# vpariza/open-hummingbird-eval

Measured on AMD Instinct MI355X. Metric: query-patches/sec, higher is better.
Workload: dtype f32

## Files before the change

### open-hummingbird-eval_amd/csrc/hbird_knn_f16.hip

```cpp
#include "hbird_knn_dev.h"
#include "hbird_rerank_dev.h"
#include <algorithm>

typedef _Float16 f16x8 __attribute__((ext_vector_type(8)));


__global__ __launch_bounds__(256) void tiles_to_f16_kernel(const float* __restrict__ t32, int g8, _Float16* __restrict__ t16,
                                                           int g16, int64_t n_row_tiles, int64_t rt0, int* __restrict__ overflow) {
    const int64_t gid = (int64_t)blockIdx.x * 256 + threadIdx.x;
    const int64_t total = n_row_tiles * g16 * 64;
    if (gid >= total) return;
    const int i = (int)(gid & 31), h = (int)((gid >> 5) & 1);
    const int64_t blk = gid >> 6;
    const int g = (int)(blk % g16);
    const int64_t rt = rt0 + blk / g16;
    f16x8 out;
#pragma unroll
    for (int j = 0; j < 8; ++j) {
        const int k = 16 * g + 8 * h + j;
        const int gg = k >> 3, kk = k & 7;
        float v = 0.0f;
        if (gg < g8) v = t32[((rt * g8) + gg) * HB_BLK + ((kk & 1) * 32 + i) * 4 + (kk >> 1)];
        out[j] = (_Float16)v;
        if (overflow && fabsf(v) > 65504.0f && fabsf(v) < INFINITY) *overflow = 1;
    }
    reinterpret_cast<f16x8*>(t16)[(rt * g16 + g) * 64 + h * 32 + i] = out;
}

int hb_launch_tiles_to_f16(const float* t32, int g8, _Float16* t16, int g16, int64_t n_row_tiles, int64_t rt0, int* overflow,
                           hipStream_t s) {
    const int64_t total = n_row_tiles * g16 * 64;
    if (total == 0) return 0;
    tiles_to_f16_kernel<<<dim3((unsigned)((total + 255) / 256)), dim3(256), 0, s>>>(t32, g8, t16, g16, n_row_tiles, rt0, overflow);
    HB_HIP(hipGetLastError());
    return 0;
}

#define F2_RING 8
#define F2_SLOT 16384
#define F2_BINIT (F2_RING * F2_SLOT)
#define F2_SCRATCH (F2_BINIT + 2048)
#define F2_PCNT (F2_SCRATCH + 8192)
#define F2_CLWORDS (F2_PCNT + 1024)
#define F2_LDS_TOTAL (F2_CLWORDS + 64)
static_assert(F2_LDS_TOTAL <= 160 * 1024, "LDS budget");

#define F2_DMA(SRC, LDS_ADDR, VOFF)                                                                                          \
    asm volatile("s_mov_b32 m0, %2\n\ts_nop 0\n\tglobal_load_lds_dwordx4 %0, %1" :: "v"(VOFF), "s"(SRC), "s"(LDS_ADDR) : "memory", "m0");
#define F2_BL(REG, SRC, OFF) asm volatile("global_load_dwordx4 %0, %1, %2 offset:" #OFF : "+v"(REG) : "v"(lane_off), "s"(SRC) : "memory");

template <int EMAX>
__global__ __launch_bounds__(HB_THREADS, 2) void knn_f16v2_kernel(knn16_args a) {
    extern __shared__ __attribute__((aligned(16))) char smem[];
    const int tid = threadIdx.x;
    const int lane = tid & 63;
    const int w = __builtin_amdgcn_readfirstlane(tid >> 6);
    const int h = lane >> 5;
    float* sc = reinterpret_cast<float*>(smem + F2_SCRATCH) + w * 256;
    int* pcnt = reinterpret_cast<int*>(smem + F2_PCNT);
    const int g16 = a.g16;
    const int NS = g16 / 2;
    const int myq = w * 32 + (lane & 31);
    const unsigned lane_off = (unsigned)lane * 16u;
    const unsigned lds_0 = (unsigned)(size_t)(__attribute__((address_space(3))) char*)smem;
    const unsigned lds_w = lds_0 + (unsigned)w * 2048u;
    cl_sync cs = cl_init(a.wg_member, a.prog, a.cl, a.lag, blockIdx.x, w == 0, smem + F2_CLWORDS);

    wg_stamp<knn16_args>(0);
    const int seg_begin = a.wg_off[blockIdx.x], seg_end = a.wg_end[blockIdx.x];
    if (w == 0) cl_publish(cs, seg_begin < seg_end ? a.segs[seg_begin].tile0 * NS : 0x7FFFFFFF, lane);
    for (int si = seg_begin; si < seg_end; ++si) {
        const hb_seg seg = HB_KARG(knn16_args, segs)[si];
        const int k = HB_KARG(knn16_args, k), klw = HB_KARG(knn16_args, klw);
        float* wl_s = HB_KARG(knn16_args, state_s) + (size_t)seg.slot * HB_QT * klw;
        unsigned* wl_i = HB_KARG(knn16_args, state_i) + (size_t)seg.slot * HB_QT * klw;
        float thr;
        {
            const knn_args_pool_view pv{HB_KARG(knn16_args, state_cnt), HB_KARG(knn16_args, state_thr)};
            thr = pool_begin(pv, seg.slot, seg.first, pcnt, myq, lane);
            thr = fmaxf(thr, floor_load(HB_KARG(knn16_args, gthr), seg.q_tile * HB_QT + myq));
        }
        const int total = seg.n_tiles * NS, clock0 = seg.tile0 * NS;
        f32x16 acc[8];
        f16x8 fa[8];
        f16x8 bq[4][2];

        const char* const qbase = reinterpret_cast<const char*>(a.q16) + (size_t)(seg.q_tile * 8 + w) * g16 * 1024;
        const char* qf = qbase;
        const char* qf1 = qbase;
        const char* bf = reinterpret_cast<const char*>(a.bank16) + ((size_t)seg.b_tile0 * 8 + w) * g16 * 1024;
        const float* bi = a.binit + (size_t)seg.b_tile0 * HB_BT;
        const long long b_wrap = ((long long)seg.stride * 8 - 1) * g16 * 1024;
        const int bi_step = seg.stride * HB_BT;
        int fks = 0, left = total;
        unsigned slot_f = 0, fpar = 0;
#define F2_REQ_B0(U) F2_BL(bq[U][0], qf, 0)
#define F2_REQ_B1(U) F2_BL(bq[U][1], qf1, 1024)
#define F2_REQ_C(I) F2_DMA(bf, lds_w + slot_f + (I) * 1024u, lane_off + (I) * 1024u)
#define F2_ADVANCE()                                                                                                         \
        {                                                                                                                    \
            if (fks == 0 && w == 0) F2_DMA(bi, lds_0 + F2_BINIT + fpar, lane_off)                                            \
            qf1 = qf;                                                                                                        \
            if (--left > 0) {                                                                                                \
                qf += 2048; bf += 2048;                                                                                      \
                if (++fks == NS) { fks = 0; qf = qbase; bf += b_wrap; bi += bi_step; fpar ^= 1024u; }                        \
            }                                                                                                                \
            slot_f = (slot_f + F2_SLOT) & (F2_RING * F2_SLOT - 1);                                                           \
        }
        F2_REQ_B0(0) F2_REQ_C(0) F2_REQ_C(1) F2_ADVANCE() F2_REQ_B1(0)
        F2_REQ_B0(1) F2_REQ_C(0) F2_REQ_C(1) F2_ADVANCE() F2_REQ_B1(1)
        F2_REQ_B0(2) F2_REQ_C(0) F2_REQ_C(1) F2_ADVANCE() F2_REQ_B1(2)
        F2_REQ_B0(3) F2_REQ_C(0) F2_REQ_C(1) F2_ADVANCE()
        asm volatile("s_waitcnt vmcnt(11)" : "+v"(bq[0][0]), "+v"(bq[0][1]) :: "memory");
        __syncthreads();
        unsigned slot_c = 0;
        int ks = 0, bt = seg.b_tile0, cpar = 0;
        bool bulk = seg.tile0 < 16;
#define F2_INIT_TILE()                                                                                                       \
        {                                                                                                                    \
            const f32x4* bi_ = reinterpret_cast<const f32x4*>(smem + F2_BINIT + cpar * 1024);                                \
            _Pragma("unroll") for (int t = 0; t < 8; ++t)                                                                    \
                _Pragma("unroll") for (int g = 0; g < 4; ++g) {                                                              \
                    const f32x4 v = bi_[8 * t + 2 * g + h];                                                                  \
                    acc[t][4 * g + 0] = v[0]; acc[t][4 * g + 1] = v[1]; acc[t][4 * g + 2] = v[2]; acc[t][4 * g + 3] = v[3]; \
                }                                                                                                            \
        }
        {
            const f16x8* A = reinterpret_cast<const f16x8*>(smem) + lane;
#pragma unroll
            for (int t = 0; t < 8; ++t) fa[t] = A[(t * 2) * 64];
        }
        F2_INIT_TILE()
#define F2_MM(T, B) acc[T] = __builtin_amdgcn_mfma_f32_32x32x16_f16(fa[T], B, acc[T], 0, 0, 0);
#define F2_STAGE(U)                                                                                                          \
        {                                                                                                                    \
            const f16x8* Ac = reinterpret_cast<const f16x8*>(smem + slot_c) + lane;                                          \
            const unsigned slot_n = (slot_c + F2_SLOT) & (F2_RING * F2_SLOT - 1);                                            \
            const f16x8* An = reinterpret_cast<const f16x8*>(smem + slot_n) + lane;                                          \
                                       \
            KN_FENCE F2_MM(0, bq[U][0]) KN_FENCE fa[0] = Ac[(0 * 2 + 1) * 64]; F2_REQ_B1((U + 3) & 3)                           \
            KN_FENCE F2_MM(1, bq[U][0]) KN_FENCE fa[1] = Ac[(1 * 2 + 1) * 64];                                                  \
            KN_FENCE F2_MM(2, bq[U][0]) KN_FENCE fa[2] = Ac[(2 * 2 + 1) * 64];                                                  \
            KN_FENCE F2_MM(3, bq[U][0]) KN_FENCE fa[3] = Ac[(3 * 2 + 1) * 64];                                                  \
            KN_FENCE F2_MM(4, bq[U][0]) KN_FENCE fa[4] = Ac[(4 * 2 + 1) * 64];                                                  \
            KN_FENCE F2_MM(5, bq[U][0]) KN_FENCE fa[5] = Ac[(5 * 2 + 1) * 64];                                                  \
            KN_FENCE F2_MM(6, bq[U][0]) KN_FENCE fa[6] = Ac[(6 * 2 + 1) * 64];                                                  \
            KN_FENCE F2_MM(7, bq[U][0]) KN_FENCE fa[7] = Ac[(7 * 2 + 1) * 64];                                                  \
            KN_FENCE                                                                                                         \
                                \
            asm volatile("s_waitcnt vmcnt(8)" : "+v"(bq[(U + 1) & 3][0]), "+v"(bq[(U + 1) & 3][1]), "+v"(bq[U][1]) :: "memory"); \
            __builtin_amdgcn_s_barrier();      \
                 \
            if ((U) == 0 && w == 0) cl_tick(cs, clock0 + st, lane);    \
            KN_FENCE F2_MM(0, bq[U][1]) KN_FENCE fa[0] = An[(0 * 2) * 64]; F2_REQ_B0(U)                                         \
            KN_FENCE F2_MM(1, bq[U][1]) KN_FENCE fa[1] = An[(1 * 2) * 64];                                                      \
            KN_FENCE F2_MM(2, bq[U][1]) KN_FENCE fa[2] = An[(2 * 2) * 64]; F2_REQ_C(0)                                          \
            KN_FENCE F2_MM(3, bq[U][1]) KN_FENCE fa[3] = An[(3 * 2) * 64];                                                      \
            KN_FENCE F2_MM(4, bq[U][1]) KN_FENCE fa[4] = An[(4 * 2) * 64]; F2_REQ_C(1)                                          \
            KN_FENCE F2_MM(5, bq[U][1]) KN_FENCE fa[5] = An[(5 * 2) * 64];                                                      \
            KN_FENCE F2_MM(6, bq[U][1]) KN_FENCE fa[6] = An[(6 * 2) * 64];                                                      \
            KN_FENCE F2_MM(7, bq[U][1]) KN_FENCE fa[7] = An[(7 * 2) * 64];                                                      \
            KN_FENCE                                                                                                         \
            F2_ADVANCE()                                                                                                     \
            KN_FENCE                                                                                                         \
            slot_c = slot_n;                                                                                                 \
        }
        for (int st = 0; st < total; st += 4) {
            F2_STAGE(0) F2_STAGE(1) F2_STAGE(2) F2_STAGE(3)
            ks += 4;
            if (ks == NS) {
                if (seg.first && bt == seg.b_tile0 && cold_start_needed(thr)) thr = fmaxf(thr, cold_start_threshold(acc, k));
                pool_epilogue_scan<EMAX>(acc, thr, wl_s, wl_i, sc, w * 32, lane, k, (unsigned)bt, klw, pcnt, bulk);
                ks = 0; bt += seg.stride; cpar ^= 1;
                F2_INIT_TILE()
                {
                    const f16x8* A = reinterpret_cast<const f16x8*>(smem + slot_c) + lane;
#pragma unroll
                    for (int t = 0; t < 8; ++t) fa[t] = A[(t * 2) * 64];
                }
            }
        }
        asm volatile("s_waitcnt vmcnt(0)" : "+v"(bq[0][0]), "+v"(bq[0][1]), "+v"(bq[1][0]), "+v"(bq[1][1]), "+v"(bq[2][0]), "+v"(bq[2][1]),
                     "+v"(bq[3][0]), "+v"(bq[3][1]) :: "memory");
#undef F2_STAGE
#undef F2_MM
#undef F2_INIT_TILE
#undef F2_ADVANCE
#undef F2_REQ_B0
#undef F2_REQ_B1
#undef F2_REQ_C
        if (w == 0) cl_publish(cs, seg.next_tile0 == 0x7FFFFFFF ? 0x7FFFFFFF : seg.next_tile0 * NS, lane);
        {
            const knn_args_pool_view pv{HB_KARG(knn16_args, state_cnt), HB_KARG(knn16_args, state_thr)};
            pool_end(pv, seg.slot, pcnt, thr, myq, lane);
        }
        if (lane < 32) floor_publish(HB_KARG(knn16_args, gthr), seg.q_tile * HB_QT + myq, thr);
        asm volatile("s_waitcnt vmcnt(0)" ::: "memory");
        __syncthreads();
    }
    cl_finish(cs, a.cl_stats, w == 0, lane);
    wg_stamp<knn16_args>(1);
}

#define HB_RERANK_PARAMS                                                                                                     \
    const float* __restrict__ binit, int d, const float* __restrict__ q, const float* __restrict__ qn2,                      \
    const int64_t* __restrict__ cand, const float* __restrict__ cand_score, const float* __restrict__ qnorm,                \
    const float* __restrict__ bmax, unsigned char* __restrict__ certified, int kc, int64_t nq, int k, int64_t id_base,      \
    int metric, int out_metric, int64_t ntotal, int64_t* __restrict__ out_idx, float* __restrict__ out_dist,                \
    hb_rerank_seeds sd, hb_centre_view cv

template <bool CENTRED>
__global__ __launch_bounds__(256) void rerank_kernel(const float* __restrict__ tiles, int g8, HB_RERANK_PARAMS) {
    __shared__ float s_sc[4][256];
    __shared__ int64_t s_id[4][256];
    const int lane = threadIdx.x & 63, wv = threadIdx.x >> 6;
    const int64_t qi = (int64_t)blockIdx.x * 4 + wv;
    if (qi >= nq) return;
    const float* qr = q + qi * (int64_t)d;
    const hb_rerank_query qc = hb_rerank_query_of<CENTRED>(qi, qnorm, bmax, d, metric, cv, cand, cand_score, kc, k);
    for (int c = lane; c < kc; c += 64) {
        const int64_t row = cand[qi * (int64_t)kc + c];
        float acc = -INFINITY;
        if (hb_rerank_needs_score(row, c, k, cand_score + qi * (int64_t)kc, qc.cut)) {
            acc = binit[row];
            const float* base = tiles + ((row >> 5) * (int64_t)g8) * HB_BLK + (int)(row & 31) * 4;
            for (int g = 0; g < g8; ++g) {
                const f32x4 e = *reinterpret_cast<const f32x4*>(base + (int64_t)g * HB_BLK);
                const f32x4 o = *reinterpret_cast<const f32x4*>(base + (int64_t)g * HB_BLK + 128);
                const int k0 = 8 * g;
#pragma unroll
                for (int j = 0; j < 4; ++j) {
                    if (k0 + 2 * j < d) acc = fmaf(qr[k0 + 2 * j], e[j], acc);
                    if (k0 + 2 * j + 1 < d) acc = fmaf(qr[k0 + 2 * j + 1], o[j], acc);
                }
            }
        }
        s_sc[wv][c] = acc;
        s_id[wv][c] = row;
    }
    __builtin_amdgcn_s_waitcnt(0xc07f);
    hb_rerank_tail<CENTRED>(s_sc[wv], s_id[wv], lane, qi, qc.E, qc.cq, cand, cand_score, qnorm, qn2, certified, kc, k, id_base, out_metric, ntotal, out_idx, out_dist, sd, cv);
}

__global__ __launch_bounds__(256) void tiles_to_rows_kernel(const float* __restrict__ t32, int g8, float* __restrict__ rows, int rs,
                                                            int64_t rt0) {
    __shared__ float s[4 * HB_BLK];
    const int64_t rt = rt0 + blockIdx.x;
    const int g0 = blockIdx.y * 4, ng = min(4, g8 - g0);
    const int t = threadIdx.x;
    if (t < ng * 64) reinterpret_cast<f32x4*>(s)[t] = reinterpret_cast<const f32x4*>(t32 + (rt * g8 + g0) * HB_BLK)[t];
    __syncthreads();
    const int i = t >> 3, c = t & 7;
    f32x4 out;
#pragma unroll
    for (int j = 0; j < 4; ++j) {
        const int kq = 4 * c + j, gl = kq >> 3, kk = kq & 7;
        out[j] = gl < ng ? s[gl * HB_BLK + ((kk & 1) * 32 + i) * 4 + (kk >> 1)] : 0.0f;
    }
    if (8 * g0 + 4 * c < rs) *reinterpret_cast<f32x4*>(rows + (rt * 32 + i) * (int64_t)rs + 8 * g0 + 4 * c) = out;
}

int hb_launch_tiles_to_row_copy(const float* t32, int g8, float* rows, int rs, int64_t n_row_tiles, int64_t rt0, hipStream_t s) {
    if (n_row_tiles <= 0) return 0;
    tiles_to_rows_kernel<<<dim3((unsigned)n_row_tiles, (unsigned)((rs / 8 + 3) / 4)), dim3(256), 0, s>>>(t32, g8, rows, rs, rt0);
    HB_HIP(hipGetLastError());
    return 0;
}

#define RRW_STRIDE 36
template <bool CENTRED>
__global__ __launch_bounds__(256) void rerank_rows_kernel(const float* __restrict__ rows, int rs, HB_RERANK_PARAMS) {
    __shared__ float s_sc[4][256];
    __shared__ unsigned s_id[4][256];
    __shared__ int s_act[4][256];
    __shared__ __attribute__((aligned(16))) float s_img[4][66 * RRW_STRIDE];
    const int lane = threadIdx.x & 63, wv = threadIdx.x >> 6;
    const int64_t qi = (int64_t)blockIdx.x * 4 + wv;
    if (qi >= nq) return;
    const float* qr = q + qi * (int64_t)d;
    const hb_rerank_query qc = hb_rerank_query_of<CENTRED>(qi, qnorm, bmax, d, metric, cv, cand, cand_score, kc, k);
    int n_act = 0;
    for (int c0 = 0; c0 < kc; c0 += 64) {
        const int c = c0 + lane;
        int64_t row = -1;
        bool act = false;
        if (c < kc) {
            row = cand[qi * (int64_t)kc + c];
            act = hb_rerank_needs_score(row, c, k, cand_score + qi * (int64_t)kc, qc.cut);
            s_sc[wv][c] = -INFINITY;
            s_id[wv][c] = row >= 0 ? (unsigned)row : HB_ID_NONE;
        }
        const unsigned long long m = __ballot(act);
        if (act) s_act[wv][n_act + __popcll(m & ((1ull << lane) - 1ull))] = c;
        n_act += __popcll(m);
    }
    __builtin_amdgcn_s_waitcnt(0xc07f);
    __builtin_amdgcn_wave_barrier();
    float* img = s_img[wv];
    const int rr = lane >> 3, chn = lane & 7;
    const int nch = (d + 31) >> 5;
    for (int b0 = 0; b0 < n_act; b0 += 64) {
        const int nb = min(64, n_act - b0);
        const int nj = (nb + 1 + 7) >> 3;
        const int c = lane < nb ? s_act[wv][b0 + lane] : -1;
        float acc = c >= 0 ? binit[s_id[wv][c]] : 0.0f;
        const float* src[9];
#pragma unroll
        for (int j = 0; j < 9; ++j) {
            const int li = 8 * j + rr;
            src[j] = li < nb ? rows + (int64_t)s_id[wv][s_act[wv][b0 + li]] * rs + 4 * chn : (li == nb ? qr + 4 * chn : nullptr);
        }
        f32x4 R[9];
#define RRW_LOAD(CH)                                                                                                         \
        _Pragma("unroll") for (int j = 0; j < 9; ++j) {                                                                      \
            if (j < nj) {                                                                                                    \
                R[j] = f32x4{0.f, 0.f, 0.f, 0.f};                                                                            \
                if (src[j]) {                                                                                                \
                    const int k0 = 32 * (CH) + 4 * chn;                                                                      \
                    if (8 * j + rr < nb || k0 + 4 <= d) R[j] = *reinterpret_cast<const f32x4*>(src[j] + 32 * (CH));          \
                    else { _Pragma("unroll") for (int e = 0; e < 4; ++e) if (k0 + e < d) R[j][e] = src[j][32 * (CH) + e]; }   \
                }                                                                                                            \
            }                                                                                                                \
        }
        RRW_LOAD(0)
        for (int ch = 0; ch < nch; ++ch) {
#pragma unroll
            for (int j = 0; j < 9; ++j)
                if (j < nj && 8 * j + rr <= nb) *reinterpret_cast<f32x4*>(img + (8 * j + rr) * RRW_STRIDE + 4 * chn) = R[j];
            if (ch + 1 < nch) { RRW_LOAD(ch + 1) }
            __builtin_amdgcn_s_waitcnt(0xc07f);
            __builtin_amdgcn_wave_barrier();
            if (c >= 0) {
                const f32x4* xr = reinterpret_cast<const f32x4*>(img + lane * RRW_STRIDE);
                const f32x4* qv = reinterpret_cast<const f32x4*>(img + nb * RRW_STRIDE);
                if (32 * ch + 32 <= d) {
#pragma unroll
                    for (int i = 0; i < 8; ++i) {
                        const f32x4 x = xr[i], y = qv[i];
                        acc = fmaf(y[0], x[0], acc); acc = fmaf(y[1], x[1], acc); acc = fmaf(y[2], x[2], acc); acc = fmaf(y[3], x[3], acc);
                    }
                } else {
                    for (int i = 0; 32 * ch + i < d; ++i) acc = fmaf(img[nb * RRW_STRIDE + i], img[lane * RRW_STRIDE + i], acc);
                }
            }
            __builtin_amdgcn_wave_barrier();
        }
#undef RRW_LOAD
        if (c >= 0) s_sc[wv][c] = acc;
    }
    __builtin_amdgcn_s_waitcnt(0xc07f);
    __builtin_amdgcn_wave_barrier();
    hb_rerank_tail<CENTRED>(s_sc[wv], s_id[wv], lane, qi, qc.E, qc.cq, cand, cand_score, qnorm, qn2, certified, kc, k, id_base, out_metric, ntotal, out_idx, out_dist, sd, cv);
}
#undef HB_RERANK_PARAMS

int hb_launch_rerank(const hb_rerank_args& a, const float* tiles, int g8, const float* rows, int rs, hipStream_t s) {
    if (a.nq == 0) return 0;
    if (a.kc > 256) return hb_fail("hb_index_search: too many candidates for the re-rank kernel");
    const bool centred = a.cv.cq != nullptr;
    auto fn = rows ? (centred ? rerank_rows_kernel<true> : rerank_rows_kernel<false>) : (centred ? rerank_kernel<true> : rerank_kernel<false>);
    fn<<<dim3((unsigned)((a.nq + 3) / 4)), dim3(256), 0, s>>>(rows ? rows : tiles, rows ? rs : g8, a.binit, a.d, a.q, a.qn2, a.cand, a.cand_score, a.qnorm, a.bmax,
                                                            a.certified, a.kc, a.nq, a.k, a.id_base, a.metric, a.out_metric, a.ntotal, a.out_idx, a.out_dist, a.sd, a.cv);
    HB_HIP(hipGetLastError());
    return 0;
}

int hb_knn_f16_launch(const knn16_args& args, int grid, hipStream_t s) {
    void (*fn)(knn16_args) = args.klw <= 256 ? knn_f16v2_kernel<4> : knn_f16v2_kernel<8>;
    if (args.klw > 512) return hb_fail("hb_index_search: candidate pools beyond 512 entries");
    if (hb_ensure_dyn_lds((const void*)fn, F2_LDS_TOTAL)) return -1;
    fn<<<dim3((unsigned)grid), dim3(HB_THREADS), F2_LDS_TOTAL, s>>>(args);
    HB_HIP(hipGetLastError());
    return 0;
}

__global__ __launch_bounds__(256) void bnorm_max_kernel(const float* __restrict__ bnorm, int64_t n, float* __restrict__ bmax) {
    float m = 0.0f;
    for (int64_t i = (int64_t)blockIdx.x * 256 + threadIdx.x; i < n; i += (int64_t)gridDim.x * 256) m = fmaxf(m, bnorm[i]);
    for (int o = 32; o > 0; o >>= 1) m = fmaxf(m, __shfl_xor(m, o));
    if ((threadIdx.x & 63) == 0) atomicMax(reinterpret_cast<int*>(bmax), __float_as_int(m));
}

int hb_launch_bnorm_max(const float* bnorm, int64_t n, float* bmax, hipStream_t s) {
    if (n == 0) return 0;
    const int64_t blocks = std::min<int64_t>((n + 255) / 256, 1024);
    bnorm_max_kernel<<<dim3((unsigned)blocks), dim3(256), 0, s>>>(bnorm, n, bmax);
    HB_HIP(hipGetLastError());
    return 0;
}

__global__ __launch_bounds__(256) void scatter_rows_kernel(const int64_t* __restrict__ rows, int64_t n, int k,
                                                           const int64_t* __restrict__ src_idx, const float* __restrict__ src_dist,
                                                           int64_t* __restrict__ out_idx, float* __restrict__ out_dist) {
    const int64_t t = (int64_t)blockIdx.x * 256 + threadIdx.x;
    if (t >= n * k) return;
    const int64_t i = t / k;
    const int j = (int)(t % k);
    out_idx[rows[i] * k + j] = src_idx[t];
    out_dist[rows[i] * k + j] = src_dist[t];
}

int hb_launch_scatter_rows(const int64_t* rows, int64_t n, int k, const int64_t* src_idx, const float* src_dist,
                           int64_t* out_idx, float* out_dist, hipStream_t s) {
    if (n == 0) return 0;
    scatter_rows_kernel<<<dim3((unsigned)((n * k + 255) / 256)), dim3(256), 0, s>>>(rows, n, k, src_idx, src_dist, out_idx, out_dist);
    HB_HIP(hipGetLastError());
    return 0;
}
```

Measured before the change: 79270.

## Switch kNN f16 kernel from 32x32x16 to 16x16x32 MFMA with permlane fixup

```diff
diff --git a/open-hummingbird-eval_amd/csrc/hbird_knn_f16.hip b/open-hummingbird-eval_amd/csrc/hbird_knn_f16.hip
--- a/open-hummingbird-eval_amd/csrc/hbird_knn_f16.hip
+++ b/open-hummingbird-eval_amd/csrc/hbird_knn_f16.hip
@@ -47,7 +47,19 @@
 
 #define F2_DMA(SRC, LDS_ADDR, VOFF)                                                                                          \
     asm volatile("s_mov_b32 m0, %2\n\ts_nop 0\n\tglobal_load_lds_dwordx4 %0, %1" :: "v"(VOFF), "s"(SRC), "s"(LDS_ADDR) : "memory", "m0");
-#define F2_BL(REG, SRC, OFF) asm volatile("global_load_dwordx4 %0, %1, %2 offset:" #OFF : "+v"(REG) : "v"(lane_off), "s"(SRC) : "memory");
+#define F2_BL(REG, SRC, OFF) asm volatile("global_load_dwordx4 %0, %1, %2 offset:" #OFF : "+v"(REG) : "v"(q_off), "s"(SRC) : "memory");
+
+template <int Q>
+__device__ __forceinline__ void f2_mm16(f32x16& acc, const f16x8& a, const f16x8& b) {
+    f32x4 c = {acc[4 * Q], acc[4 * Q + 1], acc[4 * Q + 2], acc[4 * Q + 3]};
+    c = __builtin_amdgcn_mfma_f32_16x16x32_f16(a, b, c, 0, 0, 0);
+    acc[4 * Q] = c[0]; acc[4 * Q + 1] = c[1]; acc[4 * Q + 2] = c[2]; acc[4 * Q + 3] = c[3];
+}
+template <int X, int Y>
+__device__ __forceinline__ void f2_swap16(f32x16& acc) {
+    const auto r = __builtin_amdgcn_permlane16_swap(__float_as_uint(acc[X]), __float_as_uint(acc[Y]), false, false);
+    acc[X] = __uint_as_float(r[0]); acc[Y] = __uint_as_float(r[1]);
+}
 
 template <int EMAX>
 __global__ __launch_bounds__(HB_THREADS, 2) void knn_f16v2_kernel(knn16_args a) {
@@ -55,13 +67,16 @@
     const int tid = threadIdx.x;
     const int lane = tid & 63;
     const int w = __builtin_amdgcn_readfirstlane(tid >> 6);
-    const int h = lane >> 5;
+    const int c4 = lane >> 4, m16 = lane & 15;
     float* sc = reinterpret_cast<float*>(smem + F2_SCRATCH) + w * 256;
     int* pcnt = reinterpret_cast<int*>(smem + F2_PCNT);
     const int g16 = a.g16;
     const int NS = g16 / 2;
     const int myq = w * 32 + (lane & 31);
     const unsigned lane_off = (unsigned)lane * 16u;
+    const unsigned q_off = (unsigned)((c4 >> 1) * 1024 + ((c4 & 1) * 32 + m16) * 16);
+    const unsigned a_off = (unsigned)((c4 >> 1) * 1024 + ((c4 & 1) * 32 + 8 * ((m16 >> 2) & 1) + 4 * (m16 >> 3) + (m16 & 3)) * 16);
+    const int ri = 2 * (c4 & 1) + (c4 >> 1);
     const unsigned lds_0 = (unsigned)(size_t)(__attribute__((address_space(3))) char*)smem;
     const unsigned lds_w = lds_0 + (unsigned)w * 2048u;
     cl_sync cs = cl_init(a.wg_member, a.prog, a.cl, a.lag, blockIdx.x, w == 0, smem + F2_CLWORDS);
@@ -87,7 +102,6 @@
 
         const char* const qbase = reinterpret_cast<const char*>(a.q16) + (size_t)(seg.q_tile * 8 + w) * g16 * 1024;
         const char* qf = qbase;
-        const char* qf1 = qbase;
         const char* bf = reinterpret_cast<const char*>(a.bank16) + ((size_t)seg.b_tile0 * 8 + w) * g16 * 1024;
         const float* bi = a.binit + (size_t)seg.b_tile0 * HB_BT;
         const long long b_wrap = ((long long)seg.stride * 8 - 1) * g16 * 1024;
@@ -95,23 +109,22 @@
         int fks = 0, left = total;
         unsigned slot_f = 0, fpar = 0;
 #define F2_REQ_B0(U) F2_BL(bq[U][0], qf, 0)
-#define F2_REQ_B1(U) F2_BL(bq[U][1], qf1, 1024)
+#define F2_REQ_B1(U) F2_BL(bq[U][1], qf, 256)
 #define F2_REQ_C(I) F2_DMA(bf, lds_w + slot_f + (I) * 1024u, lane_off + (I) * 1024u)
 #define F2_ADVANCE()                                                                                                         \
         {                                                                                                                    \
             if (fks == 0 && w == 0) F2_DMA(bi, lds_0 + F2_BINIT + fpar, lane_off)                                            \
-            qf1 = qf;                                                                                                        \
             if (--left > 0) {                                                                                                \
                 qf += 2048; bf += 2048;                                                                                      \
                 if (++fks == NS) { fks = 0; qf = qbase; bf += b_wrap; bi += bi_step; fpar ^= 1024u; }                        \
             }                                                                                                                \
             slot_f = (slot_f + F2_SLOT) & (F2_RING * F2_SLOT - 1);                                                           \
         }
-        F2_REQ_B0(0) F2_REQ_C(0) F2_REQ_C(1) F2_ADVANCE() F2_REQ_B1(0)
-        F2_REQ_B0(1) F2_REQ_C(0) F2_REQ_C(1) F2_ADVANCE() F2_REQ_B1(1)
-        F2_REQ_B0(2) F2_REQ_C(0) F2_REQ_C(1) F2_ADVANCE() F2_REQ_B1(2)
-        F2_REQ_B0(3) F2_REQ_C(0) F2_REQ_C(1) F2_ADVANCE()
-        asm volatile("s_waitcnt vmcnt(11)" : "+v"(bq[0][0]), "+v"(bq[0][1]) :: "memory");
+        F2_REQ_C(0) F2_REQ_C(1) F2_REQ_B0(0) F2_REQ_B1(0) F2_ADVANCE()
+        F2_REQ_C(0) F2_REQ_C(1) F2_REQ_B0(1) F2_REQ_B1(1) F2_ADVANCE()
+        F2_REQ_C(0) F2_REQ_C(1) F2_REQ_B0(2) F2_REQ_B1(2) F2_ADVANCE()
+        F2_REQ_C(0) F2_REQ_C(1) F2_REQ_B0(3) F2_REQ_B1(3) F2_ADVANCE()
+        asm volatile("s_waitcnt vmcnt(12)" : "+v"(bq[0][0]), "+v"(bq[0][1]) :: "memory");
         __syncthreads();
         unsigned slot_c = 0;
         int ks = 0, bt = seg.b_tile0, cpar = 0;
@@ -120,46 +133,53 @@
         {                                                                                                                    \
             const f32x4* bi_ = reinterpret_cast<const f32x4*>(smem + F2_BINIT + cpar * 1024);                                \
             _Pragma("unroll") for (int t = 0; t < 8; ++t)                                                                    \
-                _Pragma("unroll") for (int g = 0; g < 4; ++g) {                                                              \
-                    const f32x4 v = bi_[8 * t + 2 * g + h];                                                                  \
-                    acc[t][4 * g + 0] = v[0]; acc[t][4 * g + 1] = v[1]; acc[t][4 * g + 2] = v[2]; acc[t][4 * g + 3] = v[3]; \
+                _Pragma("unroll") for (int f = 0; f < 2; ++f) {                                                              \
+                    const f32x4 v = bi_[8 * t + 4 * f + ri];                                                                 \
+                    _Pragma("unroll") for (int j = 0; j < 4; ++j) { acc[t][8 * f + j] = v[j]; acc[t][8 * f + 4 + j] = v[j]; } \
                 }                                                                                                            \
         }
+#define F2_SWAP_TILE()                                                                                                       \
+        _Pragma("unroll") for (int t = 0; t < 8; ++t) {                                                                      \
+            f2_swap16<0, 4>(acc[t]); f2_swap16<1, 5>(acc[t]); f2_swap16<2, 6>(acc[t]); f2_swap16<3, 7>(acc[t]);              \
+            f2_swap16<8, 12>(acc[t]); f2_swap16<9, 13>(acc[t]); f2_swap16<10, 14>(acc[t]); f2_swap16<11, 15>(acc[t]);        \
+        }
+#define F2_FRAG(BASE, F) (*reinterpret_cast<const f16x8*>((BASE) + ((F) >> 1) * 2048 + ((F) & 1) * 256))
         {
-            const f16x8* A = reinterpret_cast<const f16x8*>(smem) + lane;
-#pragma unroll
-            for (int t = 0; t < 8; ++t) fa[t] = A[(t * 2) * 64];
+            const char* A = smem + a_off;
+#pragma unroll
+            for (int i = 0; i < 8; ++i) fa[i] = F2_FRAG(A, i);
         }
         F2_INIT_TILE()
-#define F2_MM(T, B) acc[T] = __builtin_amdgcn_mfma_f32_32x32x16_f16(fa[T], B, acc[T], 0, 0, 0);
+#define F2_MM(F, U) f2_mm16<2 * ((F) & 1)>(acc[(F) >> 1], fa[(F) & 7], bq[U][0]); f2_mm16<2 * ((F) & 1) + 1>(acc[(F) >> 1], fa[(F) & 7], bq[U][1]);
 #define F2_STAGE(U)                                                                                                          \
         {                                                                                                                    \
-            const f16x8* Ac = reinterpret_cast<const f16x8*>(smem + slot_c) + lane;                                          \
+            const char* Ac = smem + slot_c + a_off;                                                                          \
             const unsigned slot_n = (slot_c + F2_SLOT) & (F2_RING * F2_SLOT - 1);                                            \
-            const f16x8* An = reinterpret_cast<const f16x8*>(smem + slot_n) + lane;                                          \
-                                       \
-            KN_FENCE F2_MM(0, bq[U][0]) KN_FENCE fa[0] = Ac[(0 * 2 + 1) * 64]; F2_REQ_B1((U + 3) & 3)                           \
-            KN_FENCE F2_MM(1, bq[U][0]) KN_FENCE fa[1] = Ac[(1 * 2 + 1) * 64];                                                  \
-            KN_FENCE F2_MM(2, bq[U][0]) KN_FENCE fa[2] = Ac[(2 * 2 + 1) * 64];                                                  \
-            KN_FENCE F2_MM(3, bq[U][0]) KN_FENCE fa[3] = Ac[(3 * 2 + 1) * 64];                                                  \
-            KN_FENCE F2_MM(4, bq[U][0]) KN_FENCE fa[4] = Ac[(4 * 2 + 1) * 64];                                                  \
-            KN_FENCE F2_MM(5, bq[U][0]) KN_FENCE fa[5] = Ac[(5 * 2 + 1) * 64];                                                  \
-            KN_FENCE F2_MM(6, bq[U][0]) KN_FENCE fa[6] = Ac[(6 * 2 + 1) * 64];                                                  \
-            KN_FENCE F2_MM(7, bq[U][0]) KN_FENCE fa[7] = Ac[(7 * 2 + 1) * 64];                                                  \
+            const char* An = smem + slot_n + a_off;                                                                          \
+                                                                    \
+            KN_FENCE F2_MM(0, U) KN_FENCE fa[0] = F2_FRAG(Ac, 8);                                                               \
+            KN_FENCE F2_MM(1, U) KN_FENCE fa[1] = F2_FRAG(Ac, 9);                                                               \
+            KN_FENCE F2_MM(2, U) KN_FENCE fa[2] = F2_FRAG(Ac, 10);                                                              \
+            KN_FENCE F2_MM(3, U) KN_FENCE fa[3] = F2_FRAG(Ac, 11);                                                              \
+            KN_FENCE F2_MM(4, U) KN_FENCE fa[4] = F2_FRAG(Ac, 12);                                                              \
+            KN_FENCE F2_MM(5, U) KN_FENCE fa[5] = F2_FRAG(Ac, 13);                                                              \
+            KN_FENCE F2_MM(6, U) KN_FENCE fa[6] = F2_FRAG(Ac, 14);                                                              \
+            KN_FENCE F2_MM(7, U) KN_FENCE fa[7] = F2_FRAG(Ac, 15);                                                              \
             KN_FENCE                                                                                                         \
                                 \
-            asm volatile("s_waitcnt vmcnt(8)" : "+v"(bq[(U + 1) & 3][0]), "+v"(bq[(U + 1) & 3][1]), "+v"(bq[U][1]) :: "memory"); \
+            asm volatile("s_waitcnt vmcnt(8)" : "+v"(bq[(U + 1) & 3][0]), "+v"(bq[(U + 1) & 3][1]) :: "memory");             \
             __builtin_amdgcn_s_barrier();      \
-                 \
+             \
+                                                             \
             if ((U) == 0 && w == 0) cl_tick(cs, clock0 + st, lane);    \
-            KN_FENCE F2_MM(0, bq[U][1]) KN_FENCE fa[0] = An[(0 * 2) * 64]; F2_REQ_B0(U)                                         \
-            KN_FENCE F2_MM(1, bq[U][1]) KN_FENCE fa[1] = An[(1 * 2) * 64];                                                      \
-            KN_FENCE F2_MM(2, bq[U][1]) KN_FENCE fa[2] = An[(2 * 2) * 64]; F2_REQ_C(0)                                          \
-            KN_FENCE F2_MM(3, bq[U][1]) KN_FENCE fa[3] = An[(3 * 2) * 64];                                                      \
-            KN_FENCE F2_MM(4, bq[U][1]) KN_FENCE fa[4] = An[(4 * 2) * 64]; F2_REQ_C(1)                                          \
-            KN_FENCE F2_MM(5, bq[U][1]) KN_FENCE fa[5] = An[(5 * 2) * 64];                                                      \
-            KN_FENCE F2_MM(6, bq[U][1]) KN_FENCE fa[6] = An[(6 * 2) * 64];                                                      \
-            KN_FENCE F2_MM(7, bq[U][1]) KN_FENCE fa[7] = An[(7 * 2) * 64];                                                      \
+            KN_FENCE F2_MM(8, U) KN_FENCE fa[0] = F2_FRAG(An, 0);                                                               \
+            KN_FENCE F2_MM(9, U) KN_FENCE fa[1] = F2_FRAG(An, 1);                                                               \
+            KN_FENCE F2_MM(10, U) KN_FENCE fa[2] = F2_FRAG(An, 2); F2_REQ_C(0)                                                  \
+            KN_FENCE F2_MM(11, U) KN_FENCE fa[3] = F2_FRAG(An, 3);                                                              \
+            KN_FENCE F2_MM(12, U) KN_FENCE fa[4] = F2_FRAG(An, 4); F2_REQ_C(1)                                                  \
+            KN_FENCE F2_MM(13, U) KN_FENCE fa[5] = F2_FRAG(An, 5);                                                              \
+            KN_FENCE F2_MM(14, U) KN_FENCE fa[6] = F2_FRAG(An, 6);                                                              \
+            KN_FENCE F2_MM(15, U) KN_FENCE fa[7] = F2_FRAG(An, 7); F2_REQ_B0(U) F2_REQ_B1(U)                                    \
             KN_FENCE                                                                                                         \
             F2_ADVANCE()                                                                                                     \
             KN_FENCE                                                                                                         \
@@ -169,14 +189,15 @@
             F2_STAGE(0) F2_STAGE(1) F2_STAGE(2) F2_STAGE(3)
             ks += 4;
             if (ks == NS) {
+                F2_SWAP_TILE()
                 if (seg.first && bt == seg.b_tile0 && cold_start_needed(thr)) thr = fmaxf(thr, cold_start_threshold(acc, k));
                 pool_epilogue_scan<EMAX>(acc, thr, wl_s, wl_i, sc, w * 32, lane, k, (unsigned)bt, klw, pcnt, bulk);
                 ks = 0; bt += seg.stride; cpar ^= 1;
                 F2_INIT_TILE()
                 {
-                    const f16x8* A = reinterpret_cast<const f16x8*>(smem + slot_c) + lane;
-#pragma unroll
-                    for (int t = 0; t < 8; ++t) fa[t] = A[(t * 2) * 64];
+                    const char* A = smem + slot_c + a_off;
+#pragma unroll
+                    for (int i = 0; i < 8; ++i) fa[i] = F2_FRAG(A, i);
                 }
             }
         }
@@ -184,6 +205,8 @@
                      "+v"(bq[3][0]), "+v"(bq[3][1]) :: "memory");
 #undef F2_STAGE
 #undef F2_MM
+#undef F2_FRAG
+#undef F2_SWAP_TILE
 #undef F2_INIT_TILE
 #undef F2_ADVANCE
 #undef F2_REQ_B0
```

New measurement: 83870, median of 6. 5.8% higher.
